# toverainc/willow-inference-server

Measured on NVIDIA H100. Metric: Whisper large-v2 realtime multiple (audio s / s), beam 5, 3.84 s utterance, higher is better.
Workload: dtype f16

## Files before the change

willow_inference_server_b200/_lib.py:

```python
from __future__ import annotations

import ctypes as C
import os

import numpy as np

HERE = os.path.dirname(os.path.abspath(__file__))
LIB_PATH = os.path.join(HERE, "libwisb200.so")

N_DIMS = 20
DIM_NAMES = [
    "d_model", "n_heads", "n_enc_layers", "n_dec_layers", "n_vocab", "n_vocab_pad", "n_text_ctx", "n_mels",
    "n_audio_ctx", "sot", "eot", "transcribe", "translate", "no_timestamps", "sot_prev", "sot_lm", "no_speech",
    "blank", "lang_first", "n_langs",
]
PCM_F32, PCM_S16 = 0, 1
EPI_F16, EPI_F16_GELU, EPI_RESID_F32, EPI_CONV2, EPI_CROSSKV, EPI_F32, EPI_QKV_VT, EPI_DEC_QKV = range(8)

_lib = None

_SIGS = {
    "wisb_abi_version": (C.c_int, []),
    "wisb_last_error": (C.c_char_p, []),
    "wisb_create": (C.c_int, [C.c_char_p, C.c_int, C.POINTER(C.c_void_p)]),
# ... 240 lines not shown
    def debug_align_post(self, weights, width: int = 7, dtw_only: bool = False):
        w = np.ascontiguousarray(weights, np.float32)
        if dtw_only:
            w = w.reshape((1,) + w.shape[-2:])
        A, R, F = w.shape
        mat = np.zeros((R, F), np.float32)
        path = np.zeros((R + F, 2), np.int32)
        plen = np.zeros(1, np.int32)
        check(lib().wisb_debug_align_post(self._h, ptr(w), A, R, F, int(width), 1 if dtw_only else 0, ptr(mat), ptr(path),
                                          ptr(plen)))
        return mat, path[: plen[0]].copy()

    def debug_gemm(self, a16: np.ndarray, w16: np.ndarray, impl: int = 0, bn: int = 0, *, mode: int = EPI_F32,
                   planner: int = 0, bias=None, pos=None, out=None, aux=None, aux2=None, row_slot=None, row_pos=None,
                   a_wrap: int = 0, k_splits: int = 1, m_valid: int = 0, n_valid: int = 0, ldo: int = 0, d_model: int = 0,
                   n_heads: int = 0, batch: int = 0, kv_swizzle: int = 0, t_cap: int = 0, return_plan: bool = False):
        a16 = np.ascontiguousarray(a16, np.float16)
        w16 = np.ascontiguousarray(w16, np.float16)
        N, K = w16.shape
        M = a16.shape[0] - (1 if a_wrap else 0)
        if a16.shape[1] != (a_wrap if a_wrap else K):
            raise ValueError("A and W disagree on K")
        if out is None:
            if mode != EPI_F32 or k_splits != 1 or planner == 2:
                raise ValueError("this epilogue needs an explicit out buffer")
            out = np.zeros((M, N), np.float32)
        for buf in (out, aux, aux2):
            if buf is not None and not buf.flags["C_CONTIGUOUS"]:
                raise ValueError("out / aux / aux2 must be C-contiguous")
        bias = None if bias is None else np.ascontiguousarray(bias, np.float32)
        pos = None if pos is None else np.ascontiguousarray(pos, np.float32)
        if bias is not None and bias.size != N:
            raise ValueError("bias must have N elements")
        if pos is not None and pos.size != 1500 * (ldo or N):
            raise ValueError("pos must be [1500, ldo]")
        slot = None if row_slot is None else np.ascontiguousarray(row_slot, np.int32)
        rpos = None if row_pos is None else np.ascontiguousarray(row_pos, np.int32)
        if (slot is not None and slot.size != M) or (rpos is not None and rpos.size != M):
            raise ValueError("row_slot / row_pos must have M entries")
        prm = np.asarray([M, N, K, impl, bn, planner, mode, a_wrap, k_splits, m_valid, n_valid, ldo, d_model, n_heads, batch,
                          kv_swizzle, t_cap], np.int32)
        plan = np.zeros(4, np.int32)
        nbytes = lambda b: 0 if b is None else b.nbytes
        check(lib().wisb_debug_gemm(self._h, ptr(prm), prm.size, ptr(a16), ptr(w16), ptr(bias), ptr(pos), ptr(slot), ptr(rpos),
                                    ptr(out), out.nbytes, ptr(aux), nbytes(aux), ptr(aux2), nbytes(aux2), ptr(plan)))
        if return_plan:
            return out, dict(zip(("bn", "mcast", "k_splits", "grid"), (int(v) for v in plan)))
        return out

    def debug_search_step(self, logits, hist, mask, *, beam: int, gen: int, eot: int, no_timestamps: int,
                          timestamps: bool, max_initial_timestamp_index: int = 50, cum=None, done=None):
        logits = np.ascontiguousarray(logits, np.float32)
        R, V = logits.shape
        if R % beam:
            raise ValueError("logits rows must be n_utt * beam")
        n_utt = R // beam
        hist = np.ascontiguousarray(np.asarray(hist, np.int32).reshape(R, gen))
        mask = np.ascontiguousarray(mask, np.uint8)
        if mask.shape != (V,):
            raise ValueError("mask must have V entries")
        cum = None if cum is None else np.ascontiguousarray(cum, np.float32).reshape(R)
        done = None if done is None else np.ascontiguousarray(done, np.int32).reshape(n_utt)
# ... 65 lines not shown
```

willow_inference_server_b200/csrc/engine.cu:

```cuda
#include <stdio.h>
#include <string.h>

#include <algorithm>
#include <functional>
#include <map>
#include <memory>
#include <mutex>
#include <string>
#include <vector>

#include "../../include/wisb200.h"
#include "decoder.cuh"
#include "kernels.h"

namespace wisb {

namespace {

thread_local std::string g_last_error;

struct TensorRef {
  const uint8_t* ptr = nullptr;
  int dtype = 0, ndim = 0;
  long long shape[4] = {1, 1, 1, 1};
// ... 81 lines not shown
  int use_graphs = 1, attn_v_mn = 1, attn_ref = 0, decode_poll = 1, decoder_mega = 1;
  DevBuf<float> lm_tables;
  DevBuf<unsigned> lm_max;
  DevBuf<uint8_t> pcm_dev;
  DevBuf<long long> pcm_off;
  DevBuf<int> pcm_n;
  DevBuf<float> mel;
  int mel_B = 0;
  int enc_cap = 0;
  DevBuf<__half> h1, xn, qkv, vt, ctx, hbuf, enc_out, ckv;
  DevBuf<float> x;
  GemmPlan plan_conv2, plan_ckv;
  CUtensorMap ckv_map;
  std::vector<EncLayerPlans> enc_plans;
  AttnPlan attn_plan;
  int plans_B = 0, plans_vmn = -1, plans_pdl = -1;
  DevBuf<float> dx, dq, dctx, dh, logits;
  DevBuf<__half> dctx16, dh16, dxn16, dq16;
  DevBuf<float> dxstat;
  DevBuf<__half> kcache, vcache;
  DevBuf<uint8_t> mask_base, mask_cur;
  std::vector<int> mask_extra;
  DevBuf<float> row_lse, cum, cand_score, best_score, lang_probs, part_max, part_sum;
  DevBuf<unsigned long long> part;
  DevBuf<int> cand_idx, tokens, seq0, seq1, ind0, ind1, flip, done, n_hyp, best_len, best_tokens, prompt_dev, lang_ids;
  DevBuf<DecState> st;
  DevBuf<int> row_pos, row_slot, max_new_u;
  int search_rows = 0;
  int search_gen = 0, bd_search_gen = -1;
  int batch_rows = 320, batch_pdl = 1, decoder_batch = 1, mega_barrier = 1, cross_tc = 1, debug_chunk = 1;
  int bd_rows = 0, bd_tcap = 0, bd_launches_step = 0;
  DevBuf<float> bx, bq, bpart, blogits;
  DevBuf<__half> bxn, bctx, bh, bkc, bvc;
  std::vector<BatchLayer> bd_layers;
  GemmPlan bd_vocab;
  DevBuf<MegaLayer> mega_layers;
  DevBuf<__half> mega_img;
  int enc_pdl = 1;
  int mega_tc = 1, mega_dbg = 0;
  DevBuf<unsigned> mega_flags;
  int encoder_cache = 0;
  std::vector<float> mel_cache;
  int mel_cache_B = 0;
  bool enc_valid = false;
  int ckv_sw = 0, ckv_is_sw = 0;
  DevBuf<float> cross_part;
  DevBuf<unsigned> cross_flags;
  DevBuf<float> ln_fold;
  DevBuf<__half> fc2_chunked;
  std::vector<int> al_layer_off;
  int al_A = 0;
  DevBuf<int> al_items, al_head, al_ntext, al_nframes, al_text, al_path, al_len;
  DevBuf<float> al_cap, al_mat, al_probs;
// ... 334 lines not shown
    h->plans_B = 0;
    drop_graphs(h);
    h->h1.release();
    h->h1.ensure((static_cast<size_t>(B) * H1_ROWS + 8) * d, true);
    h->x.ensure(M * d, true);
    h->xn.ensure(M * d, true);
    h->qkv.ensure(M * 3 * d, true);
    h->vt.ensure(M * d, true);
    h->ctx.ensure(M * d, true);
    h->hbuf.ensure(M * 4 * d, true);
    h->enc_out.ensure(M * d, true);
    h->ckv.ensure(static_cast<size_t>(dm.n_dec_layers) * 2 * M * d, true);
    make_tmap_f16_2d(&h->ckv_map, h->ckv.p, HEAD_DIM, static_cast<long long>(h->ckv.n / HEAD_DIM), HEAD_DIM, HEAD_DIM, 128);
    h->enc_cap = B;
  }
  if (h->plans_B == B && h->plans_vmn == h->attn_v_mn && h->plans_pdl == h->enc_pdl) return;
  const int Mi = static_cast<int>(M);
  {
    GemmEpi e;
    e.mode = EPI_CONV2;
    e.bias = h->F("enc.conv2.b");
    e.out = h->x.p;
    e.ldo = d;
    e.pos = h->F("enc.pos");
    gemm_plan(h->plan_conv2, h->h1.p, 2LL * d, h->H("enc.conv2.w"), Mi, d, 3 * d, e, h->num_sms, 0, 2 * d);
  }
  h->enc_plans.assign(dm.n_enc_layers, EncLayerPlans());
  for (int i = 0; i < dm.n_enc_layers; ++i) {
    const std::string p = "enc." + std::to_string(i) + ".";
    EncLayerPlans& pl = h->enc_plans[i];
    GemmEpi e;
    e.mode = h->attn_v_mn ? EPI_F16 : EPI_QKV_VT;
    e.bias = h->F(p + "qkv.b");
    e.out = h->qkv.p;
    e.ldo = 3 * d;
    e.aux = h->vt.p;
    e.d_model = d;
    e.n_heads = H;
    e.batch = B;
    gemm_plan(pl.qkv, h->xn.p, d, h->H(p + "qkv.w"), Mi, 3 * d, d, e, h->num_sms);
    GemmEpi eo;
    eo.mode = EPI_RESID_F32;
    eo.bias = h->F(p + "o.b");
    eo.out = h->x.p;
    eo.ldo = d;
    gemm_plan(pl.o, h->ctx.p, d, h->H(p + "o.w"), Mi, d, d, eo, h->num_sms);
    GemmEpi e1;
    e1.mode = EPI_F16_GELU;
    e1.bias = h->F(p + "fc1.b");
    e1.out = h->hbuf.p;
    e1.ldo = 4 * d;
    gemm_plan(pl.fc1, h->xn.p, d, h->H(p + "fc1.w"), Mi, 4 * d, d, e1, h->num_sms);
    GemmEpi e2;
    e2.mode = EPI_RESID_F32;
    e2.bias = h->F(p + "fc2.b");
    e2.out = h->x.p;
    e2.ldo = d;
    gemm_plan(pl.fc2, h->hbuf.p, 4LL * d, h->H(p + "fc2.w"), Mi, d, 4 * d, e2, h->num_sms);
  }
  {
    GemmEpi e;
    e.mode = EPI_CROSSKV;
    e.bias = h->F("dec.crosskv.b");
    e.out = h->ckv.p;
    e.d_model = d;
    e.n_heads = H;
    e.batch = B;
    gemm_plan(h->plan_ckv, h->enc_out.p, d, h->H("dec.crosskv.w"), Mi, dm.n_dec_layers * 2 * d, d, e, h->num_sms);
  }
  enc_attn_plan(h->attn_plan, h->qkv.p, h->vt.p, h->ctx.p, B, d, H, h->attn_v_mn != 0);
  h->attn_plan.pdl = h->enc_pdl != 0;
  h->plan_conv2.pdl = h->plan_ckv.pdl = h->enc_pdl;
  for (EncLayerPlans& pl : h->enc_plans) pl.qkv.pdl = pl.o.pdl = pl.fc1.pdl = pl.fc2.pdl = h->enc_pdl;
  h->plans_pdl = h->enc_pdl;
  h->plans_B = B;
  h->plans_vmn = h->attn_v_mn;
}

bool want_ckv_swizzle(const wisb_handle* h, int rows) {
  return rows <= DEC_MAX_ROWS && h->decoder_batch != 2 && h->decoder_mega && h->mega_tc;
}

void run_encoder(wisb_handle* h, int B, int n_layers, bool with_ckv, int mel_first = 0) {
  const Dims& dm = h->dims;
  const int d = dm.d_model;
  const int M = B * T_ENC_PAD;
  cudaStream_t s = h->stream;
  ensure_encoder(h, B);
  h->enc_valid = false;
// ... 956 lines not shown
    WISB_REQUIRE(key != nullptr, "key is NULL");
    const std::string k(key);
    if (k == "use_graphs") h->use_graphs = value;
    else if (k == "attn_v_mn_major") h->attn_v_mn = value;
    else if (k == "attn_ref") h->attn_ref = value;
    else if (k == "decode_poll") h->decode_poll = value < 1 ? 1 : value;
    else if (k == "profile") h->profile = value;
    else if (k == "decoder_mega") h->decoder_mega = value;
    else if (k == "encoder_cache") {
      h->encoder_cache = value ? 1 : 0;
      h->enc_valid = false;
    }
    else if (k == "mega_trace") h->mega_trace_on = value;
    else if (k == "mega_dbg") h->mega_dbg = value;
    else if (k == "enc_pdl") h->enc_pdl = value ? 1 : 0;
    else if (k == "mega_trace_cta") h->mega_trace_cta = value;
    else if (k == "mega_trace_layer") h->mega_trace_layer = value;
    else if (k == "batch_rows") {
      WISB_REQUIRE(value >= 8 && value <= 1024, "batch_rows must be in [8, 1024]");
      h->batch_rows = value;
    }
    else if (k == "batch_pdl") h->batch_pdl = value ? 1 : 0;
    else if (k == "mega_barrier") h->mega_barrier = value ? 1 : 0;
    else if (k == "debug_chunk") h->debug_chunk = value;
    else if (k == "mega_tc" || k == "mega_mma") {
      WISB_REQUIRE(!value || h->mega_img.p != nullptr, "mega_mma needs d_model <= 1280 and a multiple of 64");
      h->mega_tc = value ? 1 : 0;
    }
    else if (k == "cross_tc") {
      h->cross_tc = value ? 1 : 0;
// ... 221 lines not shown
        const float* p = h->pin_f.p + u * nl;
        std::stable_sort(order.begin(), order.end(), [&](int a, int b) { return p[a] > p[b]; });
        for (int i = 0; i < nl; ++i) {
          lang_ids_out[static_cast<size_t>(u0 + u) * nl + i] = ids[order[i]];
          probs_out[static_cast<size_t>(u0 + u) * nl + i] = p[order[i]];
        }
      }
    }
  });
}

int wisb_debug_gemm(wisb_handle* h, const int32_t* prm, int n_prm, const uint16_t* a, const uint16_t* w, const float* bias,
                    const float* pos, const int32_t* row_slot, const int32_t* row_pos, void* out, size_t out_bytes, void* aux,
                    size_t aux_bytes, void* aux2, size_t aux2_bytes, int32_t* plan_out) {
  return guarded(h, [&] {
    WISB_REQUIRE(prm != nullptr && n_prm == 17 && a && w && out, "debug_gemm: bad arguments");
    const int M = prm[0], N = prm[1], K = prm[2], impl = prm[3], bn = prm[4], planner = prm[5], a_wrap = prm[7],
              k_splits = prm[8];
    GemmEpi e;
    e.mode = prm[6];
    e.m_valid = prm[9] > 0 ? prm[9] : M;
    e.n_valid = prm[10] > 0 ? prm[10] : N;
    e.ldo = prm[11] > 0 ? prm[11] : N;
    e.d_model = prm[12];
    e.n_heads = prm[13];
    e.batch = prm[14];
    e.kv_swizzle = prm[15];
    e.t_cap = prm[16];
    WISB_REQUIRE(M > 0 && N > 0 && K > 0 && a_wrap >= 0 && k_splits >= 1 && impl >= 0 && impl <= 1 && planner >= 0 && planner <= 2,
                 "debug_gemm: bad scalar parameters");
    WISB_REQUIRE(e.mode >= EPI_F16 && e.mode <= EPI_DEC_QKV, "debug_gemm: unknown epilogue");
    WISB_REQUIRE(e.m_valid <= M && e.n_valid <= N && e.n_valid % 32 == 0 && e.ldo >= e.n_valid, "debug_gemm: bad m_valid / n_valid / ldo");
    WISB_REQUIRE(planner == 0 || (a_wrap == 0 && k_splits == 1 && bn == 0), "debug_gemm: the decoder planner picks BN and the split itself");
    WISB_REQUIRE(impl == 0 || (e.mode == EPI_F32 && planner == 0 && a_wrap == 0 && k_splits == 1), "debug_gemm: the SIMT check computes plain F32 only");
    cudaStream_t s = h->stream;
    const long long lda = a_wrap > 0 ? a_wrap : K;
    const size_t a_elems = static_cast<size_t>(a_wrap > 0 ? M + 1 : M) * lda;
    DevBuf<__half> da, dw;
    DevBuf<float> dbias, dpos;
    DevBuf<int> dslot, dpos_row;
    DevBuf<uint8_t> dout, daux, daux2;
    da.ensure(a_elems);
    dw.ensure(static_cast<size_t>(N) * K);
    WISB_CUDA(cudaMemcpyAsync(da.p, a, sizeof(__half) * a_elems, cudaMemcpyHostToDevice, s));
    WISB_CUDA(cudaMemcpyAsync(dw.p, w, sizeof(__half) * N * K, cudaMemcpyHostToDevice, s));
    if (bias) {
      dbias.ensure(N);
      WISB_CUDA(cudaMemcpyAsync(dbias.p, bias, sizeof(float) * N, cudaMemcpyHostToDevice, s));
// ... 42 lines not shown
        for (size_t r = 0; r < mv; ++r) {
          WISB_REQUIRE(row_slot[r] >= 0 && row_pos[r] >= 0 && row_pos[r] < e.t_cap, "debug_gemm: row slot / position out of range");
          const size_t end = (static_cast<size_t>(row_slot[r]) * e.t_cap + row_pos[r] + 1) * d * 2;
          if (end > top) top = end;
        }
        need_aux = need_aux2 = top;
        dslot.ensure(M);
        dpos_row.ensure(M);
        WISB_CUDA(cudaMemcpyAsync(dslot.p, row_slot, sizeof(int) * M, cudaMemcpyHostToDevice, s));
        WISB_CUDA(cudaMemcpyAsync(dpos_row.p, row_pos, sizeof(int) * M, cudaMemcpyHostToDevice, s));
        e.row_slot = dslot.p;
        e.row_pos = dpos_row.p;
      }
      if (planner == 0) {
        if (e.mode == EPI_F32) e.split_stride = static_cast<long long>(M) * e.ldo;
        gemm_plan(p, da.p, lda, dw.p, M, N, K, e, h->num_sms, bn, a_wrap, k_splits);
      } else {
        plan_dec_gemm(h, p, da.p, lda, dw.p, M, N, K, e, planner == 2);
      }
      if (p.epi.mode == EPI_F32) need_out = ((p.k_splits - 1) * static_cast<size_t>(p.epi.split_stride) + mv * e.ldo) * 4;
      WISB_REQUIRE(out_bytes >= need_out && aux_bytes >= need_aux && aux2_bytes >= need_aux2 &&
                       (need_aux == 0 || e.aux != nullptr) && (need_aux2 == 0 || e.aux2 != nullptr),
                   "debug_gemm: an output buffer is too small for the epilogue");
      gemm_run(p, s);
    }
    WISB_CUDA(cudaMemcpyAsync(out, e.out, out_bytes, cudaMemcpyDeviceToHost, s));
    if (e.aux) WISB_CUDA(cudaMemcpyAsync(aux, e.aux, aux_bytes, cudaMemcpyDeviceToHost, s));
    if (e.aux2) WISB_CUDA(cudaMemcpyAsync(aux2, e.aux2, aux2_bytes, cudaMemcpyDeviceToHost, s));
    WISB_CUDA(cudaStreamSynchronize(s));
    if (plan_out) {
      plan_out[0] = impl == 1 ? 0 : p.BN;
      plan_out[1] = impl == 1 ? 0 : p.mcast;
      plan_out[2] = impl == 1 ? 1 : p.k_splits;
      plan_out[3] = impl == 1 ? 0 : p.grid;
    }
  });
}

int wisb_debug_search_step(wisb_handle* h, const int32_t* prm, int n_prm, const float* logits, const int32_t* hist,
                           const uint8_t* mask, const float* cum, const int32_t* done, int32_t* cand_idx, float* cand_score,
                           float* row_lse) {
  return guarded(h, [&] {
    WISB_REQUIRE(prm != nullptr && n_prm == 8 && logits && mask && cand_idx && cand_score && row_lse, "debug_search_step: bad arguments");
    const int n_utt = prm[0], beam = prm[1], gen = prm[2], V = prm[3], eot = prm[4], no_ts = prm[5], ts = prm[6], max_init = prm[7];
    WISB_REQUIRE(n_utt >= 1 && n_utt <= 64 && beam >= 1 && beam <= MAX_BEAM && gen >= 0 && gen + 2 <= T_MAX && V >= 2 &&
                     eot >= 0 && eot < V && (ts == 0 || ts == 1) && max_init >= 0 && (gen == 0 || hist != nullptr),
                 "debug_search_step: bad scalar parameters");
    WISB_REQUIRE(!ts || (no_ts > eot && no_ts + 1 < V), "debug_search_step: bad timestamp geometry");
    cudaStream_t s = h->stream;
// ... 349 lines not shown
```

willow_inference_server_b200/csrc/gemm_tc.cu:

```cuda
#include <mutex>

#include "kernels.h"
#include "ptx.cuh"

namespace wisb {

namespace {

constexpr int BM = 128;
constexpr int BK = 64;
constexpr int A_STAGE_BYTES = BM * BK * 2;
constexpr int GEMM_CONSUMERS = 256;
constexpr int GEMM_THREADS = GEMM_CONSUMERS + 128;
constexpr int EPI_LD = 66, EPI_HALF = 33;
constexpr int EPI_BYTES = (GEMM_CONSUMERS / 32) * 16 * EPI_LD * 4;

template <int BN>
struct GemmCfg {
  static constexpr int STAGES = (BN == 256) ? 4 : (BN == 160 ? 5 : (BN == 128 ? 6 : 8));
  static constexpr int B_STAGE_BYTES = BN * BK * 2;
  static constexpr int SMEM_BYTES = STAGES * (A_STAGE_BYTES + B_STAGE_BYTES) + EPI_BYTES + 1024  + 256 ;
  static_assert(SMEM_BYTES <= 232448, "gemm: shared memory per block");
};

// ... 125 lines not shown
#pragma unroll
        for (int i = 0; i < 8; ++i) o4[i] = make_float4(f[4 * i + 0], f[4 * i + 1], f[4 * i + 2], f[4 * i + 3]);
      } else {
        const bool is_v = col0 >= 2 * d;
        const int c = col0 - (is_v ? 2 * d : d);
        const long long at = (static_cast<long long>(__ldg(e.row_slot + row)) * e.t_cap + __ldg(e.row_pos + row)) * d + c;
        store_f16x32(reinterpret_cast<__half*>(is_v ? e.aux2 : e.aux) + at, f);
      }
      break;
    }
    default:
      break;
  }
}

template <int BN, bool kMC>
__global__ void __launch_bounds__(GEMM_THREADS, 1)
gemm_tc_kernel(const __grid_constant__ CUtensorMap map_a, const __grid_constant__ CUtensorMap map_b, int M, int N, int K,
               int a_wrap, int k_splits, const GemmEpi epi) {
  using Cfg = GemmCfg<BN>;
  constexpr int STAGES = Cfg::STAGES;
  extern __shared__ uint8_t smem_raw[];
  const uint32_t raw_addr = smem_u32(smem_raw);
  const uint32_t base = (raw_addr + 1023u) & ~1023u;
  uint8_t* smem = smem_raw + (base - raw_addr);
  const uint32_t smem_a0 = base;
  const uint32_t smem_b0 = base + STAGES * A_STAGE_BYTES;
  float* epi_stage = reinterpret_cast<float*>(smem + STAGES * (A_STAGE_BYTES + Cfg::B_STAGE_BYTES));
  uint64_t* bars = reinterpret_cast<uint64_t*>(smem + STAGES * (A_STAGE_BYTES + Cfg::B_STAGE_BYTES) + EPI_BYTES);
  const uint32_t bar0 = smem_u32(bars);
  auto full_bar = [&](int s) { return bar0 + 8u * s; };
  auto empty_bar = [&](int s) { return bar0 + 8u * (STAGES + s); };

  const int warp = threadIdx.x >> 5;
  const int lane = threadIdx.x & 31;
  pdl_launch_dependents();
  const int n_tiles = (N + BN - 1) / BN;
  const int k_blocks = K / BK / k_splits;
  const uint32_t crank = kMC ? cluster_ctarank() : 0u;
  const int first_unit = kMC ? static_cast<int>(blockIdx.x >> 1) : static_cast<int>(blockIdx.x);
  const int unit_stride = kMC ? static_cast<int>(gridDim.x >> 1) : static_cast<int>(gridDim.x);

  if (threadIdx.x == 0) {
    for (int s = 0; s < STAGES; ++s) {
      mbar_init(full_bar(s), 1);
      mbar_init(empty_bar(s), (GEMM_CONSUMERS / 128) * (kMC ? 2 : 1));
    }
    fence_mbar_init();
    tma_prefetch_desc(&map_a);
    tma_prefetch_desc(&map_b);
  }
  __syncthreads();
  if (kMC) cluster_sync_all();
  pdl_wait();
  int m_tiles = M / BM;
  if (epi.m_dyn != nullptr) {
    const int mt = (*epi.m_dyn + BM - 1) / BM;
    if (mt < m_tiles) m_tiles = mt;
  }
  if (kMC) m_tiles = (m_tiles + 1) & ~1;
  const int m_units = kMC ? m_tiles / 2 : m_tiles;
  const int total_tiles = m_units * n_tiles * k_splits;
  auto unit_split = [&](int unit) { return unit % k_splits; };
  auto unit_m0 = [&](int unit) { return (((unit / k_splits) % m_units) * (kMC ? 2 : 1) + static_cast<int>(crank)) * BM; };
  auto unit_n0 = [&](int unit) { return ((unit / k_splits) / m_units) * BN; };

  if (warp >= GEMM_CONSUMERS / 32) {
    setmaxnreg_dec<40>();
    if (warp == GEMM_CONSUMERS / 32 && lane == 0) {
      int stage = 0;
      uint32_t phase = 0;
      for (int tile = first_unit; tile < total_tiles; tile += unit_stride) {
        const int m0 = unit_m0(tile);
        const int n0 = unit_n0(tile);
        const int kb0 = unit_split(tile) * k_blocks;
        for (int kbl = 0; kbl < k_blocks; ++kbl) {
          const int kb = kb0 + kbl;
          mbar_wait(empty_bar(stage), phase ^ 1u);
          mbar_arrive_expect_tx(full_bar(stage), A_STAGE_BYTES + Cfg::B_STAGE_BYTES);
          int ka = kb * BK, ra = m0;
          if (a_wrap > 0 && ka >= a_wrap) {
            ka -= a_wrap;
            ra += 1;
          }
          tma_load_2d(smem_a0 + stage * A_STAGE_BYTES, &map_a, full_bar(stage), ka, ra);
          if (kMC) {
            tma_load_2d_mcast(smem_b0 + stage * Cfg::B_STAGE_BYTES + crank * (Cfg::B_STAGE_BYTES / 2), &map_b, full_bar(stage),
                              kb * BK, n0 + static_cast<int>(crank) * (BN / 2), 0x3);
          } else {
            tma_load_2d(smem_b0 + stage * Cfg::B_STAGE_BYTES, &map_b, full_bar(stage), kb * BK, n0);
          }
          if (++stage == STAGES) {
            stage = 0;
            phase ^= 1u;
          }
        }
      }
    }
  } else {
    setmaxnreg_inc<232>();
    const int wg = warp >> 2;
    const bool signaller = (threadIdx.x & 127) == 0;
    auto release = [&](int s) {
      if (signaller) {
        if (kMC) {
          mbar_arrive_cluster(empty_bar(s), 0);
          mbar_arrive_cluster(empty_bar(s), 1);
        } else {
          mbar_arrive(empty_bar(s));
        }
      }
    };
    float* stg = epi_stage + warp * 16 * EPI_LD;
    int stage = 0;
    uint32_t phase = 0;
    for (int tile = first_unit; tile < total_tiles; tile += unit_stride) {
      const int m0 = unit_m0(tile);
      const int n0 = unit_n0(tile);
      const int split = unit_split(tile);
      float acc[BN / 2];
#pragma unroll
      for (int i = 0; i < BN / 2; ++i) acc[i] = 0.f;
// ... 86 lines not shown

}

void make_tmap_f16_2d(CUtensorMap* map, const void* ptr, long long cols, long long rows, long long ld, int box_cols,
                      int box_rows) {
  cuuint64_t dims[2] = {static_cast<cuuint64_t>(cols), static_cast<cuuint64_t>(rows)};
  cuuint64_t strides[1] = {static_cast<cuuint64_t>(ld) * 2};
  cuuint32_t box[2] = {static_cast<cuuint32_t>(box_cols), static_cast<cuuint32_t>(box_rows)};
  cuuint32_t estr[2] = {1, 1};
  CUresult r = get_encode_fn()(map, CU_TENSOR_MAP_DATA_TYPE_FLOAT16, 2, const_cast<void*>(ptr), dims, strides, box, estr,
                               CU_TENSOR_MAP_INTERLEAVE_NONE, CU_TENSOR_MAP_SWIZZLE_128B,
                               CU_TENSOR_MAP_L2_PROMOTION_L2_256B, CU_TENSOR_MAP_FLOAT_OOB_FILL_NONE);
  if (r != CUDA_SUCCESS) throw Error(2, "cuTensorMapEncodeTiled failed with CUresult " + std::to_string(static_cast<int>(r)));
}

void gemm_plan(GemmPlan& p, const __half* a, long long lda, const __half* w, int M, int N, int K, const GemmEpi& epi,
               int num_sms, int force_bn, int a_wrap, int k_splits) {
  WISB_REQUIRE(M > 0 && M % BM == 0, "gemm: M must be a positive multiple of 128");
  WISB_REQUIRE(K > 0 && K % BK == 0, "gemm: K must be a positive multiple of 64");
  WISB_REQUIRE(N > 0 && N % 32 == 0, "gemm: N must be a positive multiple of 32");
  WISB_REQUIRE((lda * 2) % 16 == 0 && (reinterpret_cast<uintptr_t>(a) & 15) == 0 && (reinterpret_cast<uintptr_t>(w) & 15) == 0,
               "gemm: operands must be 16-byte aligned");
  WISB_REQUIRE(k_splits >= 1 && (K / BK) % k_splits == 0, "gemm: K blocks must divide evenly over the K splits");
  WISB_REQUIRE(k_splits == 1 || (epi.mode == EPI_F32 && epi.split_stride > 0), "gemm: split-K needs the EPI_F32 partial epilogue");
  p.M = M;
  p.N = N;
  p.K = K;
  p.k_splits = k_splits;
  p.epi = epi;
  if (p.epi.m_valid <= 0) p.epi.m_valid = M;
  if (p.epi.n_valid <= 0) p.epi.n_valid = N;
  const bool no_mcast = force_bn < 0;
  int bn = force_bn < 0 ? -force_bn : force_bn;
  if (bn == 0) {
    long long best = -1;
    for (int cand : {256, 160, 128}) {
      if (N % cand != 0) continue;
      const long long t = static_cast<long long>(M / BM) * (N / cand);
      const long long cost = ((t + num_sms - 1) / num_sms) * (cand + 48);
      if (best < 0 || cost < best) {
        best = cost;
        bn = cand;
      }
    }
    if (bn == 0) bn = 128;
  }
  WISB_REQUIRE(bn == 64 || bn == 128 || bn == 160 || bn == 256, "gemm: BN must be 64, 128, 160 or 256");
  p.BN = bn;
  const int tiles = (M / BM) * ((N + bn - 1) / bn) * k_splits;
  p.mcast = (!no_mcast && (M / BM) % 2 == 0 && N % bn == 0 && a_wrap == 0 && num_sms >= 2) ? 1 : 0;
  if (p.mcast) {
    const int units = tiles / 2, clusters = num_sms / 2;
    p.grid = 2 * (units < clusters ? units : clusters);
  } else {
    p.grid = tiles < num_sms ? tiles : num_sms;
  }
  p.a_wrap = a_wrap;
  if (a_wrap > 0) {
    WISB_REQUIRE(a_wrap % BK == 0 && lda == a_wrap && K > a_wrap && K - a_wrap <= a_wrap, "gemm: bad a_wrap");
    make_tmap_f16_2d(&p.map_a, a, a_wrap, M + 1, lda, BK, BM);
  } else {
    make_tmap_f16_2d(&p.map_a, a, K, M, lda, BK, BM);
  }
  make_tmap_f16_2d(&p.map_b, w, K, N, K, BK, p.mcast ? bn / 2 : bn);
}

template <int BN, bool kMC>
void gemm_launch(const GemmPlan& p, cudaStream_t stream) {
  static std::atomic<unsigned long long> once{0};
  once_per_device(once, [] {
    WISB_CUDA(cudaFuncSetAttribute(gemm_tc_kernel<BN, kMC>, cudaFuncAttributeMaxDynamicSharedMemorySize, GemmCfg<BN>::SMEM_BYTES));
  });
  cudaLaunchConfig_t cfg{};
  cfg.gridDim = dim3(p.grid);
  cfg.blockDim = dim3(GEMM_THREADS);
  cfg.dynamicSmemBytes = GemmCfg<BN>::SMEM_BYTES;
  cfg.stream = stream;
  cudaLaunchAttribute attr[2];
  attr[0].id = cudaLaunchAttributeClusterDimension;
  attr[0].val.clusterDim.x = kMC ? 2 : 1;
  attr[0].val.clusterDim.y = 1;
  attr[0].val.clusterDim.z = 1;
  attr[1].id = cudaLaunchAttributeProgrammaticStreamSerialization;
  attr[1].val.programmaticStreamSerializationAllowed = 1;
  cfg.attrs = attr;
  cfg.numAttrs = p.pdl ? 2 : 1;
  WISB_CUDA(cudaLaunchKernelEx(&cfg, gemm_tc_kernel<BN, kMC>, p.map_a, p.map_b, p.M, p.N, p.K, p.a_wrap, p.k_splits, p.epi));
}

void gemm_run(const GemmPlan& p, cudaStream_t stream) {
  if (p.BN == 64) {
    if (p.mcast) gemm_launch<64, true>(p, stream); else gemm_launch<64, false>(p, stream);
  } else if (p.BN == 256) {
    if (p.mcast) gemm_launch<256, true>(p, stream); else gemm_launch<256, false>(p, stream);
  } else if (p.BN == 160) {
    if (p.mcast) gemm_launch<160, true>(p, stream); else gemm_launch<160, false>(p, stream);
  } else {
    if (p.mcast) gemm_launch<128, true>(p, stream); else gemm_launch<128, false>(p, stream);
  }
}

void gemm_ref_run(const __half* a, long long lda, const __half* w, float* c, int M, int N, int K, cudaStream_t stream) {
  dim3 grid(cdiv(N, 128), M);
  gemm_ref_kernel<<<grid, 128, 0, stream>>>(a, lda, w, c, M, N, K);
  WISB_CUDA(cudaGetLastError());
}

}
```

willow_inference_server_b200/csrc/kernels.h:

```cpp
#pragma once
#include "common.cuh"

namespace wisb {

enum EpiMode : int {
  EPI_F16 = 0,
  EPI_F16_GELU = 1,
  EPI_RESID_F32 = 2,
  EPI_CONV2 = 3,
  EPI_CROSSKV = 4,
  EPI_F32 = 5,
  EPI_QKV_VT = 6,
  EPI_DEC_QKV = 7,
};

struct GemmEpi {
  int mode = EPI_F16;
  const float* bias = nullptr;
  void* out = nullptr;
  long long ldo = 0;
  int m_valid = 0;
  int n_valid = 0;
  const float* pos = nullptr;
  void* aux = nullptr;
  void* aux2 = nullptr;
  int d_model = 0, n_heads = 0, batch = 0;
  int batch_off = 0;
  int kv_swizzle = 0;
  const int* row_slot = nullptr;
  const int* row_pos = nullptr;
  int t_cap = 0;
  long long split_stride = 0;
  const int* m_dyn = nullptr;
};

struct GemmPlan {
  CUtensorMap map_a, map_b;
  int M = 0, N = 0, K = 0, BN = 128, grid = 0, a_wrap = 0, mcast = 0, k_splits = 1, pdl = 0;
  GemmEpi epi;
};

void gemm_plan(GemmPlan& p, const __half* a, long long lda, const __half* w, int M, int N, int K, const GemmEpi& epi,
               int num_sms, int force_bn = 0, int a_wrap = 0, int k_splits = 1);
void gemm_run(const GemmPlan& p, cudaStream_t stream);
void gemm_ref_run(const __half* a, long long lda, const __half* w, float* c, int M, int N, int K, cudaStream_t stream);

void make_tmap_f16_2d(CUtensorMap* map, const void* ptr, long long cols, long long rows, long long ld, int box_cols,
                      int box_rows);

size_t logmel_table_floats();
void logmel_init_tables(float* tables_dev, cudaStream_t stream);
void logmel_run(const void* pcm, int pcm_is_s16, const long long* offsets_dev, const int* n_samples_dev, int B,
                const float* tables_dev, float* mel, unsigned* max_ws , cudaStream_t stream);

void conv1_gelu_run(const float* mel, const __half* w , const float* bias, __half* h1, int B, int d,
                    cudaStream_t stream);
void layernorm_f32_to_f16_run(const float* x, const float* g, const float* b, __half* y, int rows, int d,
                              cudaStream_t stream, bool pdl = false);
// ... 13 lines not shown
```

Baseline: 124.7.

## Add 2x2 multicast GEMM clusters and cost-model tile planner for encoder

```diff
diff --git a/willow_inference_server_b200/_lib.py b/willow_inference_server_b200/_lib.py
--- a/willow_inference_server_b200/_lib.py
+++ b/willow_inference_server_b200/_lib.py
@@ -278,7 +278,8 @@
     def debug_gemm(self, a16: np.ndarray, w16: np.ndarray, impl: int = 0, bn: int = 0, *, mode: int = EPI_F32,
                    planner: int = 0, bias=None, pos=None, out=None, aux=None, aux2=None, row_slot=None, row_pos=None,
                    a_wrap: int = 0, k_splits: int = 1, m_valid: int = 0, n_valid: int = 0, ldo: int = 0, d_model: int = 0,
-                   n_heads: int = 0, batch: int = 0, kv_swizzle: int = 0, t_cap: int = 0, return_plan: bool = False):
+                   n_heads: int = 0, batch: int = 0, kv_swizzle: int = 0, t_cap: int = 0, return_plan: bool = False,
+                   cluster=None):
         a16 = np.ascontiguousarray(a16, np.float16)
         w16 = np.ascontiguousarray(w16, np.float16)
         N, K = w16.shape
@@ -303,13 +304,13 @@
         if (slot is not None and slot.size != M) or (rpos is not None and rpos.size != M):
             raise ValueError("row_slot / row_pos must have M entries")
         prm = np.asarray([M, N, K, impl, bn, planner, mode, a_wrap, k_splits, m_valid, n_valid, ldo, d_model, n_heads, batch,
-                          kv_swizzle, t_cap], np.int32)
-        plan = np.zeros(4, np.int32)
+                          kv_swizzle, t_cap] + ([] if cluster is None else [cluster]), np.int32)
+        plan = np.zeros(4 if cluster is None else 5, np.int32)
         nbytes = lambda b: 0 if b is None else b.nbytes
         check(lib().wisb_debug_gemm(self._h, ptr(prm), prm.size, ptr(a16), ptr(w16), ptr(bias), ptr(pos), ptr(slot), ptr(rpos),
                                     ptr(out), out.nbytes, ptr(aux), nbytes(aux), ptr(aux2), nbytes(aux2), ptr(plan)))
         if return_plan:
-            return out, dict(zip(("bn", "mcast", "k_splits", "grid"), (int(v) for v in plan)))
+            return out, dict(zip(("bn", "mcast", "k_splits", "grid", "cluster"), (int(v) for v in plan)))
         return out
 
     def debug_search_step(self, logits, hist, mask, *, beam: int, gen: int, eot: int, no_timestamps: int,
diff --git a/willow_inference_server_b200/csrc/engine.cu b/willow_inference_server_b200/csrc/engine.cu
--- a/willow_inference_server_b200/csrc/engine.cu
+++ b/willow_inference_server_b200/csrc/engine.cu
@@ -119,7 +119,7 @@
   CUtensorMap ckv_map;
   std::vector<EncLayerPlans> enc_plans;
   AttnPlan attn_plan;
-  int plans_B = 0, plans_vmn = -1, plans_pdl = -1;
+  int plans_B = 0, plans_vmn = -1, plans_pdl = -1, plans_cluster = -1;
   DevBuf<float> dx, dq, dctx, dh, logits;
   DevBuf<__half> dctx16, dh16, dxn16, dq16;
   DevBuf<float> dxstat;
@@ -142,6 +142,7 @@
   DevBuf<MegaLayer> mega_layers;
   DevBuf<__half> mega_img;
   int enc_pdl = 1;
+  int enc_cluster = 0;
   int mega_tc = 1, mega_dbg = 0;
   DevBuf<unsigned> mega_flags;
   int encoder_cache = 0;
@@ -506,7 +507,7 @@
     make_tmap_f16_2d(&h->ckv_map, h->ckv.p, HEAD_DIM, static_cast<long long>(h->ckv.n / HEAD_DIM), HEAD_DIM, HEAD_DIM, 128);
     h->enc_cap = B;
   }
-  if (h->plans_B == B && h->plans_vmn == h->attn_v_mn && h->plans_pdl == h->enc_pdl) return;
+  if (h->plans_B == B && h->plans_vmn == h->attn_v_mn && h->plans_pdl == h->enc_pdl && h->plans_cluster == h->enc_cluster) return;
   const int Mi = static_cast<int>(M);
   {
     GemmEpi e;
@@ -530,25 +531,25 @@
     e.d_model = d;
     e.n_heads = H;
     e.batch = B;
-    gemm_plan(pl.qkv, h->xn.p, d, h->H(p + "qkv.w"), Mi, 3 * d, d, e, h->num_sms);
+    gemm_plan(pl.qkv, h->xn.p, d, h->H(p + "qkv.w"), Mi, 3 * d, d, e, h->num_sms, 0, 0, 1, h->enc_cluster);
     GemmEpi eo;
     eo.mode = EPI_RESID_F32;
     eo.bias = h->F(p + "o.b");
     eo.out = h->x.p;
     eo.ldo = d;
-    gemm_plan(pl.o, h->ctx.p, d, h->H(p + "o.w"), Mi, d, d, eo, h->num_sms);
+    gemm_plan(pl.o, h->ctx.p, d, h->H(p + "o.w"), Mi, d, d, eo, h->num_sms, 0, 0, 1, h->enc_cluster);
     GemmEpi e1;
     e1.mode = EPI_F16_GELU;
     e1.bias = h->F(p + "fc1.b");
     e1.out = h->hbuf.p;
     e1.ldo = 4 * d;
-    gemm_plan(pl.fc1, h->xn.p, d, h->H(p + "fc1.w"), Mi, 4 * d, d, e1, h->num_sms);
+    gemm_plan(pl.fc1, h->xn.p, d, h->H(p + "fc1.w"), Mi, 4 * d, d, e1, h->num_sms, 0, 0, 1, h->enc_cluster);
     GemmEpi e2;
     e2.mode = EPI_RESID_F32;
     e2.bias = h->F(p + "fc2.b");
     e2.out = h->x.p;
     e2.ldo = d;
-    gemm_plan(pl.fc2, h->hbuf.p, 4LL * d, h->H(p + "fc2.w"), Mi, d, 4 * d, e2, h->num_sms);
+    gemm_plan(pl.fc2, h->hbuf.p, 4LL * d, h->H(p + "fc2.w"), Mi, d, 4 * d, e2, h->num_sms, 0, 0, 1, h->enc_cluster);
   }
   {
     GemmEpi e;
@@ -558,13 +559,15 @@
     e.d_model = d;
     e.n_heads = H;
     e.batch = B;
-    gemm_plan(h->plan_ckv, h->enc_out.p, d, h->H("dec.crosskv.w"), Mi, dm.n_dec_layers * 2 * d, d, e, h->num_sms);
+    gemm_plan(h->plan_ckv, h->enc_out.p, d, h->H("dec.crosskv.w"), Mi, dm.n_dec_layers * 2 * d, d, e, h->num_sms, 0, 0, 1,
+              h->enc_cluster);
   }
   enc_attn_plan(h->attn_plan, h->qkv.p, h->vt.p, h->ctx.p, B, d, H, h->attn_v_mn != 0);
   h->attn_plan.pdl = h->enc_pdl != 0;
   h->plan_conv2.pdl = h->plan_ckv.pdl = h->enc_pdl;
   for (EncLayerPlans& pl : h->enc_plans) pl.qkv.pdl = pl.o.pdl = pl.fc1.pdl = pl.fc2.pdl = h->enc_pdl;
   h->plans_pdl = h->enc_pdl;
+  h->plans_cluster = h->enc_cluster;
   h->plans_B = B;
   h->plans_vmn = h->attn_v_mn;
 }
@@ -1551,6 +1554,10 @@
     else if (k == "mega_trace") h->mega_trace_on = value;
     else if (k == "mega_dbg") h->mega_dbg = value;
     else if (k == "enc_pdl") h->enc_pdl = value ? 1 : 0;
+    else if (k == "enc_cluster") {
+      WISB_REQUIRE(value == 0 || value == 1 || value == 2 || value == 4, "enc_cluster must be 0, 1, 2 or 4");
+      h->enc_cluster = value;
+    }
     else if (k == "mega_trace_cta") h->mega_trace_cta = value;
     else if (k == "mega_trace_layer") h->mega_trace_layer = value;
     else if (k == "batch_rows") {
@@ -1802,7 +1809,8 @@
                     const float* pos, const int32_t* row_slot, const int32_t* row_pos, void* out, size_t out_bytes, void* aux,
                     size_t aux_bytes, void* aux2, size_t aux2_bytes, int32_t* plan_out) {
   return guarded(h, [&] {
-    WISB_REQUIRE(prm != nullptr && n_prm == 17 && a && w && out, "debug_gemm: bad arguments");
+    WISB_REQUIRE(prm != nullptr && (n_prm == 17 || n_prm == 18) && a && w && out, "debug_gemm: bad arguments");
+    const int cluster = n_prm == 18 ? prm[17] : -1;
     const int M = prm[0], N = prm[1], K = prm[2], impl = prm[3], bn = prm[4], planner = prm[5], a_wrap = prm[7],
               k_splits = prm[8];
     GemmEpi e;
@@ -1820,6 +1828,8 @@
     WISB_REQUIRE(e.mode >= EPI_F16 && e.mode <= EPI_DEC_QKV, "debug_gemm: unknown epilogue");
     WISB_REQUIRE(e.m_valid <= M && e.n_valid <= N && e.n_valid % 32 == 0 && e.ldo >= e.n_valid, "debug_gemm: bad m_valid / n_valid / ldo");
     WISB_REQUIRE(planner == 0 || (a_wrap == 0 && k_splits == 1 && bn == 0), "debug_gemm: the decoder planner picks BN and the split itself");
+    WISB_REQUIRE(cluster == -1 || ((cluster == 0 || cluster == 1 || cluster == 2 || cluster == 4) && planner == 0),
+                 "debug_gemm: cluster must be 0, 1, 2 or 4, with the encoder planner");
     WISB_REQUIRE(impl == 0 || (e.mode == EPI_F32 && planner == 0 && a_wrap == 0 && k_splits == 1), "debug_gemm: the SIMT check computes plain F32 only");
     cudaStream_t s = h->stream;
     const long long lda = a_wrap > 0 ? a_wrap : K;
@@ -1892,7 +1902,7 @@
       }
       if (planner == 0) {
         if (e.mode == EPI_F32) e.split_stride = static_cast<long long>(M) * e.ldo;
-        gemm_plan(p, da.p, lda, dw.p, M, N, K, e, h->num_sms, bn, a_wrap, k_splits);
+        gemm_plan(p, da.p, lda, dw.p, M, N, K, e, h->num_sms, bn, a_wrap, k_splits, cluster);
       } else {
         plan_dec_gemm(h, p, da.p, lda, dw.p, M, N, K, e, planner == 2);
       }
@@ -1911,6 +1921,7 @@
       plan_out[1] = impl == 1 ? 0 : p.mcast;
       plan_out[2] = impl == 1 ? 1 : p.k_splits;
       plan_out[3] = impl == 1 ? 0 : p.grid;
+      if (n_prm == 18) plan_out[4] = impl == 1 ? 1 : p.cluster;
     }
   });
 }
diff --git a/willow_inference_server_b200/csrc/gemm_tc.cu b/willow_inference_server_b200/csrc/gemm_tc.cu
--- a/willow_inference_server_b200/csrc/gemm_tc.cu
+++ b/willow_inference_server_b200/csrc/gemm_tc.cu
@@ -163,12 +163,14 @@
   }
 }
 
-template <int BN, bool kMC>
+template <int BN, int kCL>
 __global__ void __launch_bounds__(GEMM_THREADS, 1)
 gemm_tc_kernel(const __grid_constant__ CUtensorMap map_a, const __grid_constant__ CUtensorMap map_b, int M, int N, int K,
                int a_wrap, int k_splits, const GemmEpi epi) {
   using Cfg = GemmCfg<BN>;
   constexpr int STAGES = Cfg::STAGES;
+  constexpr bool kMC = kCL > 1;
+  static_assert(kCL == 1 || kCL == 2 || kCL == 4, "gemm: cluster of 1, 2 or 4 CTAs");
   extern __shared__ uint8_t smem_raw[];
   const uint32_t raw_addr = smem_u32(smem_raw);
   const uint32_t base = (raw_addr + 1023u) & ~1023u;
@@ -187,13 +189,14 @@
   const int n_tiles = (N + BN - 1) / BN;
   const int k_blocks = K / BK / k_splits;
   const uint32_t crank = kMC ? cluster_ctarank() : 0u;
-  const int first_unit = kMC ? static_cast<int>(blockIdx.x >> 1) : static_cast<int>(blockIdx.x);
-  const int unit_stride = kMC ? static_cast<int>(gridDim.x >> 1) : static_cast<int>(gridDim.x);
+  const int mi = static_cast<int>(crank & 1u), nj = static_cast<int>(crank >> 1);
+  const int first_unit = static_cast<int>(blockIdx.x) / kCL;
+  const int unit_stride = static_cast<int>(gridDim.x) / kCL;
 
   if (threadIdx.x == 0) {
     for (int s = 0; s < STAGES; ++s) {
       mbar_init(full_bar(s), 1);
-      mbar_init(empty_bar(s), (GEMM_CONSUMERS / 128) * (kMC ? 2 : 1));
+      mbar_init(empty_bar(s), (GEMM_CONSUMERS / 128) * (kCL == 4 ? 3 : kCL));
     }
     fence_mbar_init();
     tma_prefetch_desc(&map_a);
@@ -209,10 +212,11 @@
   }
   if (kMC) m_tiles = (m_tiles + 1) & ~1;
   const int m_units = kMC ? m_tiles / 2 : m_tiles;
-  const int total_tiles = m_units * n_tiles * k_splits;
+  const int n_units = kCL == 4 ? n_tiles / 2 : n_tiles;
+  const int total_tiles = m_units * n_units * k_splits;
   auto unit_split = [&](int unit) { return unit % k_splits; };
-  auto unit_m0 = [&](int unit) { return (((unit / k_splits) % m_units) * (kMC ? 2 : 1) + static_cast<int>(crank)) * BM; };
-  auto unit_n0 = [&](int unit) { return ((unit / k_splits) / m_units) * BN; };
+  auto unit_m0 = [&](int unit) { return (((unit / k_splits) % m_units) * (kMC ? 2 : 1) + (kMC ? mi : 0)) * BM; };
+  auto unit_n0 = [&](int unit) { return (((unit / k_splits) / m_units) * (kCL == 4 ? 2 : 1) + nj) * BN; };
 
   if (warp >= GEMM_CONSUMERS / 32) {
     setmaxnreg_dec<40>();
@@ -232,10 +236,15 @@
             ka -= a_wrap;
             ra += 1;
           }
-          tma_load_2d(smem_a0 + stage * A_STAGE_BYTES, &map_a, full_bar(stage), ka, ra);
+          if (kCL == 4) {
+            tma_load_2d_mcast(smem_a0 + stage * A_STAGE_BYTES + nj * (A_STAGE_BYTES / 2), &map_a, full_bar(stage), ka,
+                              ra + nj * (BM / 2), static_cast<uint16_t>((1u << crank) | (1u << (crank ^ 2u))));
+          } else {
+            tma_load_2d(smem_a0 + stage * A_STAGE_BYTES, &map_a, full_bar(stage), ka, ra);
+          }
           if (kMC) {
-            tma_load_2d_mcast(smem_b0 + stage * Cfg::B_STAGE_BYTES + crank * (Cfg::B_STAGE_BYTES / 2), &map_b, full_bar(stage),
-                              kb * BK, n0 + static_cast<int>(crank) * (BN / 2), 0x3);
+            tma_load_2d_mcast(smem_b0 + stage * Cfg::B_STAGE_BYTES + mi * (Cfg::B_STAGE_BYTES / 2), &map_b, full_bar(stage),
+                              kb * BK, n0 + mi * (BN / 2), static_cast<uint16_t>((1u << crank) | (1u << (crank ^ 1u))));
           } else {
             tma_load_2d(smem_b0 + stage * Cfg::B_STAGE_BYTES, &map_b, full_bar(stage), kb * BK, n0);
           }
@@ -253,8 +262,9 @@
     auto release = [&](int s) {
       if (signaller) {
         if (kMC) {
-          mbar_arrive_cluster(empty_bar(s), 0);
-          mbar_arrive_cluster(empty_bar(s), 1);
+          mbar_arrive_cluster(empty_bar(s), crank);
+          mbar_arrive_cluster(empty_bar(s), crank ^ 1u);
+          if (kCL == 4) mbar_arrive_cluster(empty_bar(s), crank ^ 2u);
         } else {
           mbar_arrive(empty_bar(s));
         }
@@ -371,8 +381,92 @@
   if (r != CUDA_SUCCESS) throw Error(2, "cuTensorMapEncodeTiled failed with CUresult " + std::to_string(static_cast<int>(r)));
 }
 
+double enc_gemm_cost(int bn, int cluster, int k_blocks, int rounds) {
+  const int ci = cluster == 4 ? 2 : cluster - 1;
+  const int bi = bn == 256 ? 2 : (bn == 160 ? 1 : 0);
+  static const double per_kblock[3][3] = {
+      {0.507, 0.509, 0.645}, {0.509, 0.548, 0.669}, {0.525, 0.523, 0.669}};
+  static const double per_tile[3][3] = {{4.33, 7.60, 12.30}, {3.42, 6.04, 11.26}, {1.98, 5.70, 9.74}};
+  static const double tail[3] = {4.0, 4.0, 12.0};
+  return rounds * (k_blocks * per_kblock[ci][bi] + per_tile[ci][bi]) + tail[bi];
+}
+
+EncTileChoice enc_tile_choice(int m_tiles, int N, int k_blocks, int force_bn, int cluster, bool allow_cluster4,
+                              const int (&slots)[3][3]) {
+  EncTileChoice best;
+  const int want_bn = force_bn < 0 ? -force_bn : force_bn;
+  for (int bn : {256, 160, 128}) {
+    if (want_bn > 0 ? bn != want_bn : N % bn != 0) continue;
+    const int bi = bn == 256 ? 2 : (bn == 160 ? 1 : 0);
+    const int n_tiles = (N + bn - 1) / bn;
+    const bool whole = N % bn == 0 && m_tiles % 2 == 0 && force_bn >= 0;
+    const bool ok[3] = {true, whole, whole && allow_cluster4 && n_tiles % 2 == 0};
+    int ci_force = -1;
+    if (cluster > 0)
+      for (int ci = (cluster == 4 ? 2 : cluster - 1); ci >= 0 && ci_force < 0; --ci)
+        if (ok[ci]) ci_force = ci;
+    for (int ci = 2; ci >= 0; --ci) {
+      if (!ok[ci] || (ci_force >= 0 && ci != ci_force)) continue;
+      const int cl = ci == 2 ? 4 : ci + 1;
+      const int units = m_tiles * n_tiles / cl;
+      const int rounds = (units + slots[ci][bi] - 1) / slots[ci][bi];
+      const double cost = enc_gemm_cost(bn, cl, k_blocks, rounds);
+      if (best.bn == 0 || cost < best.cost) best = EncTileChoice{bn, cl, rounds, cost};
+    }
+  }
+  return best;
+}
+
+namespace {
+
+template <int BN, int CL>
+void gemm_prepare() {
+  static std::atomic<unsigned long long> once{0};
+  once_per_device(once, [] {
+    WISB_CUDA(cudaFuncSetAttribute(gemm_tc_kernel<BN, CL>, cudaFuncAttributeMaxDynamicSharedMemorySize, GemmCfg<BN>::SMEM_BYTES));
+  });
+}
+
+template <int BN, int CL>
+int cluster_slots() {
+  gemm_prepare<BN, CL>();
+  cudaLaunchConfig_t cfg{};
+  cfg.gridDim = dim3(CL);
+  cfg.blockDim = dim3(GEMM_THREADS);
+  cfg.dynamicSmemBytes = GemmCfg<BN>::SMEM_BYTES;
+  cudaLaunchAttribute attr[1];
+  attr[0].id = cudaLaunchAttributeClusterDimension;
+  attr[0].val.clusterDim.x = CL;
+  attr[0].val.clusterDim.y = 1;
+  attr[0].val.clusterDim.z = 1;
+  cfg.attrs = attr;
+  cfg.numAttrs = 1;
+  int n = 0;
+  WISB_CUDA(cudaOccupancyMaxActiveClusters(&n, gemm_tc_kernel<BN, CL>, &cfg));
+  WISB_REQUIRE(n > 0, "gemm: no cluster of the GEMM kernel fits on this device");
+  return n;
+}
+
+const int (&device_slots())[3][3] {
+  static int table[64][3][3];
+  static std::atomic<unsigned long long> once{0};
+  static std::mutex mu;
+  int dev = 0;
+  WISB_CUDA(cudaGetDevice(&dev));
+  std::lock_guard<std::mutex> lock(mu);
+  once_per_device(once, [&] {
+    int (&t)[3][3] = table[dev & 63];
+    t[0][0] = cluster_slots<128, 1>(), t[0][1] = cluster_slots<160, 1>(), t[0][2] = cluster_slots<256, 1>();
+    t[1][0] = cluster_slots<128, 2>(), t[1][1] = cluster_slots<160, 2>(), t[1][2] = cluster_slots<256, 2>();
+    t[2][0] = cluster_slots<128, 4>(), t[2][1] = cluster_slots<160, 4>(), t[2][2] = cluster_slots<256, 4>();
+  });
+  return table[dev & 63];
+}
+
+}
+
 void gemm_plan(GemmPlan& p, const __half* a, long long lda, const __half* w, int M, int N, int K, const GemmEpi& epi,
-               int num_sms, int force_bn, int a_wrap, int k_splits) {
+               int num_sms, int force_bn, int a_wrap, int k_splits, int cluster) {
   WISB_REQUIRE(M > 0 && M % BM == 0, "gemm: M must be a positive multiple of 128");
   WISB_REQUIRE(K > 0 && K % BK == 0, "gemm: K must be a positive multiple of 64");
   WISB_REQUIRE(N > 0 && N % 32 == 0, "gemm: N must be a positive multiple of 32");
@@ -380,54 +474,70 @@
                "gemm: operands must be 16-byte aligned");
   WISB_REQUIRE(k_splits >= 1 && (K / BK) % k_splits == 0, "gemm: K blocks must divide evenly over the K splits");
   WISB_REQUIRE(k_splits == 1 || (epi.mode == EPI_F32 && epi.split_stride > 0), "gemm: split-K needs the EPI_F32 partial epilogue");
+  WISB_REQUIRE(cluster >= -1 && cluster <= 4 && cluster != 3, "gemm: cluster must be -1, 0, 1, 2 or 4");
   p.M = M;
   p.N = N;
   p.K = K;
   p.k_splits = k_splits;
+  p.cluster = 0;
   p.epi = epi;
   if (p.epi.m_valid <= 0) p.epi.m_valid = M;
   if (p.epi.n_valid <= 0) p.epi.n_valid = N;
   const bool no_mcast = force_bn < 0;
   int bn = force_bn < 0 ? -force_bn : force_bn;
-  if (bn == 0) {
-    long long best = -1;
-    for (int cand : {256, 160, 128}) {
-      if (N % cand != 0) continue;
-      const long long t = static_cast<long long>(M / BM) * (N / cand);
-      const long long cost = ((t + num_sms - 1) / num_sms) * (cand + 48);
-      if (best < 0 || cost < best) {
-        best = cost;
-        bn = cand;
-      }
-    }
-    if (bn == 0) bn = 128;
-  }
-  WISB_REQUIRE(bn == 64 || bn == 128 || bn == 160 || bn == 256, "gemm: BN must be 64, 128, 160 or 256");
-  p.BN = bn;
-  const int tiles = (M / BM) * ((N + bn - 1) / bn) * k_splits;
-  p.mcast = (!no_mcast && (M / BM) % 2 == 0 && N % bn == 0 && a_wrap == 0 && num_sms >= 2) ? 1 : 0;
-  if (p.mcast) {
-    const int units = tiles / 2, clusters = num_sms / 2;
-    p.grid = 2 * (units < clusters ? units : clusters);
-  } else {
-    p.grid = tiles < num_sms ? tiles : num_sms;
-  }
+  const bool bn_ok = bn == 0 || bn == 64 || bn == 128 || bn == 160 || bn == 256;
+  WISB_REQUIRE(bn_ok, "gemm: BN must be 64, 128, 160 or 256");
+  if (cluster >= 0 && bn != 64 && a_wrap == 0 && num_sms >= 2) {
+    const bool allow4 = k_splits == 1 && epi.m_dyn == nullptr;
+    const EncTileChoice c = enc_tile_choice(M / BM, N, K / BK / k_splits, no_mcast ? -bn : bn, cluster, allow4, device_slots());
+    if (c.bn > 0) {
+      const int ci = c.cluster == 4 ? 2 : c.cluster - 1;
+      const int bi = c.bn == 256 ? 2 : (c.bn == 160 ? 1 : 0);
+      const int units = (M / BM) * ((N + c.bn - 1) / c.bn) * k_splits / c.cluster, slots = device_slots()[ci][bi];
+      p.BN = c.bn;
+      p.cluster = c.cluster;
+      p.grid = c.cluster * (units < slots ? units : slots);
+    }
+  }
+  if (p.cluster == 0) {
+    if (bn == 0) {
+      long long best = -1;
+      for (int cand : {256, 160, 128}) {
+        if (N % cand != 0) continue;
+        const long long t = static_cast<long long>(M / BM) * (N / cand);
+        const long long cost = ((t + num_sms - 1) / num_sms) * (cand + 48);
+        if (best < 0 || cost < best) {
+          best = cost;
+          bn = cand;
+        }
+      }
+      if (bn == 0) bn = 128;
+    }
+    p.BN = bn;
+    const int tiles = (M / BM) * ((N + bn - 1) / bn) * k_splits;
+    const bool pair = !no_mcast && (M / BM) % 2 == 0 && N % bn == 0 && a_wrap == 0 && num_sms >= 2 && cluster != 1;
+    p.cluster = pair ? 2 : 1;
+    if (pair) {
+      const int units = tiles / 2, clusters = num_sms / 2;
+      p.grid = 2 * (units < clusters ? units : clusters);
+    } else {
+      p.grid = tiles < num_sms ? tiles : num_sms;
+    }
+  }
+  p.mcast = p.cluster > 1 ? 1 : 0;
   p.a_wrap = a_wrap;
   if (a_wrap > 0) {
     WISB_REQUIRE(a_wrap % BK == 0 && lda == a_wrap && K > a_wrap && K - a_wrap <= a_wrap, "gemm: bad a_wrap");
     make_tmap_f16_2d(&p.map_a, a, a_wrap, M + 1, lda, BK, BM);
   } else {
-    make_tmap_f16_2d(&p.map_a, a, K, M, lda, BK, BM);
-  }
-  make_tmap_f16_2d(&p.map_b, w, K, N, K, BK, p.mcast ? bn / 2 : bn);
-}
-
-template <int BN, bool kMC>
+    make_tmap_f16_2d(&p.map_a, a, K, M, lda, BK, p.cluster == 4 ? BM / 2 : BM);
+  }
+  make_tmap_f16_2d(&p.map_b, w, K, N, K, BK, p.mcast ? p.BN / 2 : p.BN);
+}
+
+template <int BN, int CL>
 void gemm_launch(const GemmPlan& p, cudaStream_t stream) {
-  static std::atomic<unsigned long long> once{0};
-  once_per_device(once, [] {
-    WISB_CUDA(cudaFuncSetAttribute(gemm_tc_kernel<BN, kMC>, cudaFuncAttributeMaxDynamicSharedMemorySize, GemmCfg<BN>::SMEM_BYTES));
-  });
+  gemm_prepare<BN, CL>();
   cudaLaunchConfig_t cfg{};
   cfg.gridDim = dim3(p.grid);
   cfg.blockDim = dim3(GEMM_THREADS);
@@ -435,25 +545,33 @@
   cfg.stream = stream;
   cudaLaunchAttribute attr[2];
   attr[0].id = cudaLaunchAttributeClusterDimension;
-  attr[0].val.clusterDim.x = kMC ? 2 : 1;
+  attr[0].val.clusterDim.x = CL;
   attr[0].val.clusterDim.y = 1;
   attr[0].val.clusterDim.z = 1;
   attr[1].id = cudaLaunchAttributeProgrammaticStreamSerialization;
   attr[1].val.programmaticStreamSerializationAllowed = 1;
   cfg.attrs = attr;
   cfg.numAttrs = p.pdl ? 2 : 1;
-  WISB_CUDA(cudaLaunchKernelEx(&cfg, gemm_tc_kernel<BN, kMC>, p.map_a, p.map_b, p.M, p.N, p.K, p.a_wrap, p.k_splits, p.epi));
+  WISB_CUDA(cudaLaunchKernelEx(&cfg, gemm_tc_kernel<BN, CL>, p.map_a, p.map_b, p.M, p.N, p.K, p.a_wrap, p.k_splits, p.epi));
+}
+
+template <int BN>
+void gemm_launch_bn(const GemmPlan& p, cudaStream_t stream) {
+  if (p.cluster == 4) gemm_launch<BN, 4>(p, stream);
+  else if (p.cluster == 2) gemm_launch<BN, 2>(p, stream);
+  else gemm_launch<BN, 1>(p, stream);
 }
 
 void gemm_run(const GemmPlan& p, cudaStream_t stream) {
   if (p.BN == 64) {
-    if (p.mcast) gemm_launch<64, true>(p, stream); else gemm_launch<64, false>(p, stream);
+    WISB_REQUIRE(p.cluster != 4, "gemm: no 4-CTA clusters at BN 64");
+    if (p.cluster == 2) gemm_launch<64, 2>(p, stream); else gemm_launch<64, 1>(p, stream);
   } else if (p.BN == 256) {
-    if (p.mcast) gemm_launch<256, true>(p, stream); else gemm_launch<256, false>(p, stream);
+    gemm_launch_bn<256>(p, stream);
   } else if (p.BN == 160) {
-    if (p.mcast) gemm_launch<160, true>(p, stream); else gemm_launch<160, false>(p, stream);
+    gemm_launch_bn<160>(p, stream);
   } else {
-    if (p.mcast) gemm_launch<128, true>(p, stream); else gemm_launch<128, false>(p, stream);
+    gemm_launch_bn<128>(p, stream);
   }
 }
 
diff --git a/willow_inference_server_b200/csrc/kernels.h b/willow_inference_server_b200/csrc/kernels.h
--- a/willow_inference_server_b200/csrc/kernels.h
+++ b/willow_inference_server_b200/csrc/kernels.h
@@ -36,12 +36,20 @@
 
 struct GemmPlan {
   CUtensorMap map_a, map_b;
-  int M = 0, N = 0, K = 0, BN = 128, grid = 0, a_wrap = 0, mcast = 0, k_splits = 1, pdl = 0;
+  int M = 0, N = 0, K = 0, BN = 128, grid = 0, a_wrap = 0, mcast = 0, cluster = 1, k_splits = 1, pdl = 0;
   GemmEpi epi;
 };
 
 void gemm_plan(GemmPlan& p, const __half* a, long long lda, const __half* w, int M, int N, int K, const GemmEpi& epi,
-               int num_sms, int force_bn = 0, int a_wrap = 0, int k_splits = 1);
+               int num_sms, int force_bn = 0, int a_wrap = 0, int k_splits = 1, int cluster = -1);
+
+double enc_gemm_cost(int bn, int cluster, int k_blocks, int rounds);
+struct EncTileChoice {
+  int bn = 0, cluster = 0, rounds = 0;
+  double cost = 0.0;
+};
+EncTileChoice enc_tile_choice(int m_tiles, int N, int k_blocks, int force_bn, int cluster, bool allow_cluster4,
+                              const int (&slots)[3][3]);
 void gemm_run(const GemmPlan& p, cudaStream_t stream);
 void gemm_ref_run(const __half* a, long long lda, const __half* w, float* c, int M, int N, int K, cudaStream_t stream);
 
```

After: 125.8, median of 6. No clear change (+0.9%).
